# dmkozh/stellar-core

Measured on AMD Instinct MI355X. Metric: ed25519 verifies/sec @1M batch (1/8 GPU) + p50 latency @1k batch, higher is better.
Workload: dtype u32

## Files before the change

stellar-core_amd/csrc/ge25519.h:

```cpp
#pragma once

#include "fe25519.h"



struct ge_p2 { fe X, Y, Z; };
struct ge_p3 { fe X, Y, Z, T; };
struct ge_p1p1 { fe X, Y, Z, T; };
struct ge_cached { fe YpX, YmX, Z, T2d; };
struct ge_precomp { fe ypx, ymx, xy2d; };

SV_HD void ge_p2_identity(ge_p2& p) {
  fe_0(p.X);
  fe_1(p.Y);
  fe_1(p.Z);
}

SV_HD void ge_dbl(ge_p1p1& r, const fe& X, const fe& Y, const fe& Z) {
  fe XX, YY, ZZ2, A, AA;
  fe_add(A, X, Y);
  fe_sq(AA, A);
  fe_sq(XX, X);
  fe_sq(YY, Y);
  fe_sq2(ZZ2, Z);
  fe_add(r.Y, YY, XX);
  fe_sub(r.Z, YY, XX);
  fe_sub4(r.X, AA, r.Y);
  fe_sub4(r.T, ZZ2, r.Z);
  fe_weak_even(r.T);
}

SV_HD void ge_p1p1_convert(ge_p3& r, const ge_p1p1& p, bool wantT) {
  {
    fe19 y19;
    fe_premul19(y19, p.Y);
    if (wantT) fe_mul_g19(r.T, p.X, p.Y, y19);
    fe_mul_g19(r.Y, p.Z, p.Y, y19);
  }
  fe19 t19;
  fe_premul19(t19, p.T);
  fe_mul_g19(r.X, p.X, p.T, t19);
  fe_mul_g19(r.Z, p.Z, p.T, t19);
}

SV_HD void ge_p1p1_to_p2(ge_p2& r, const ge_p1p1& p) {
  ge_p3 t;
  ge_p1p1_convert(t, p, false);
  r.X = t.X;
  r.Y = t.Y;
  r.Z = t.Z;
}

SV_HD void ge_p1p1_to_p3(ge_p3& r, const ge_p1p1& p) { ge_p1p1_convert(r, p, true); }

SV_HD void ge_p1p1_to_p3_opt(ge_p3& r, const ge_p1p1& p, bool wantT) { ge_p1p1_convert(r, p, wantT); }

SV_HD void ge_add_preswapped(ge_p1p1& r, const ge_p3& p, const fe& qa, const fe& qb, const fe& qZ,
                             const fe& qT2d, bool neg, bool zone) {
  fe t0, t1, PP, MM, TT, ZZ2, zp, zm;
  fe_mul(TT, p.T, qT2d);
  if (zone) {
    fe_add(ZZ2, p.Z, p.Z);
    fe_weak(ZZ2);
  } else {
    fe_mul2(ZZ2, p.Z, qZ);
  }
  fe_add(t0, p.Y, p.X);
  fe_sub(t1, p.Y, p.X);
  fe_mul(PP, t0, qa);
  fe_mul(MM, t1, qb);
  fe_sub(r.X, PP, MM);
  fe_add(r.Y, PP, MM);
  fe_add(zp, ZZ2, TT);
  fe_sub(zm, ZZ2, TT);
  SV_UNROLL for (int i = 0; i < 10; ++i) {
    r.Z.v[i] = neg ? zm.v[i] : zp.v[i];
    r.T.v[i] = neg ? zp.v[i] : zm.v[i];
  }
}

SV_HD void ge_p3_to_cached(ge_cached& c, const ge_p3& p) {
  fe d2;
  fe_const_2d(d2);
  fe_add(c.YpX, p.Y, p.X);
  fe_sub(c.YmX, p.Y, p.X);
  c.Z = p.Z;
  fe_mul(c.T2d, p.T, d2);
}

SV_HD void ge_cached_identity(ge_cached& c) {
  fe_1(c.YpX);
  fe_1(c.YmX);
  fe_1(c.Z);
  fe_0(c.T2d);
}

SV_HD bool ge_frombytes_finish(ge_p3& h, const fe& u, const fe& v, const uint32_t w[8], bool negate) {
  fe vxx, chk, chk2, xs, sq;
  fe_sq(vxx, h.X);
  fe_mul(vxx, vxx, v);
  fe_sub(chk, vxx, u);
  fe_add(chk2, vxx, u);
  const bool m_ok = fe_iszero(chk);
  const bool p_ok = fe_iszero(chk2);
  fe_const_sqrtm1(sq);
  fe_mul(xs, h.X, sq);
  fe_cmov(h.X, xs, !m_ok);
  const uint32_t sign = w[7] >> 31;
  fe nx;
  fe_neg(nx, h.X);
  const bool flip = negate ? (fe_isnegative(h.X) == sign) : (fe_isnegative(h.X) != sign);
  fe_cmov(h.X, nx, flip);
  fe_weak(h.X);
  fe_mul(h.T, h.X, h.Y);
  return m_ok || p_ok;
}

SV_COLD bool ge_frombytes(ge_p3& h, const uint32_t w[8], bool negate) {
  fe u, v, v3, one, d;
  fe_1(one);
  fe_const_d(d);
  fe_frombytes(h.Y, w);
  fe_1(h.Z);
  fe_sq(u, h.Y);
  fe_mul(v, u, d);
  fe_sub(u, u, one);
  fe_weak(u);
  fe_add(v, v, one);
  fe_weak(v);
  fe_sq(v3, v);
  fe_mul(v3, v3, v);
  fe_sq(h.X, v3);
  fe_mul(h.X, h.X, v);
  fe_mul(h.X, h.X, u);
  fe_pow22523(h.X, h.X);
  fe_mul(h.X, h.X, v3);
  fe_mul(h.X, h.X, u);
  return ge_frombytes_finish(h, u, v, w, negate);
}

SV_COLD void ge_p2_tobytes_zinv(uint32_t out[8], const fe& X, const fe& Y, const fe& zi) {
  fe x, y;
  fe_mul(x, X, zi);
  fe_mul(y, Y, zi);
  fe_tobytes(out, y);
  out[7] ^= fe_isnegative(x) << 31;
}

SV_COLD void ge_p2_tobytes(uint32_t out[8], const fe& X, const fe& Y, const fe& Z) {
  fe zi;
  fe_invert(zi, Z);
  ge_p2_tobytes_zinv(out, X, Y, zi);
}
```

stellar-core_amd/csrc/sv_kernels.hip:

```cpp
#include <hip/hip_runtime.h>

#include <atomic>

#include "verify_core.h"
#include "quad.h"
#include "sv_kparams.h"
#include "keytab.h"
#include "launch.h"

#define SV_BLOCK 256
#define SV_WAVES_PER_SIMD 2
#ifndef SV_QUAD_WAVES
#define SV_QUAD_WAVES 3
#endif
#ifndef SV_MAIN_WAVES
#define SV_MAIN_WAVES 3
#endif

#define SV_DBG_TRIVIAL_PAIR 1u
#define SV_DBG_MAX_WINDOWS 2u
#define SV_DBG_PREP_ONLY 8u
#define SV_DBG_KEY_COLLIDE 16u
#define SV_DBG_DROP_HANDOVER 0x80u
__device__ __forceinline__ int sv_wave_windows(int wl, uint32_t dbg) {
// ... 85 lines not shown
      ks = (uint32_t)s;
      break;
    }
  }
  t.kslot[li] = ks;
}

__global__ __launch_bounds__(SV_BLOCK, SV_PREP_WAVES) void sv_keybuild_kernel(sv_cparams c) {
  const sv_ktparams& t = c.kt;
  const uint32_t nb = t.count[0];
  const uint64_t i = (uint64_t)blockIdx.x * blockDim.x + threadIdx.x;
  const uint32_t lane = threadIdx.x & 63u;
  if (i - lane >= nb) return;
  const bool active = i < nb;
  const uint32_t s = t.builders[active ? i : nb - 1];
  sv_u4* e = t.store + (uint64_t)s * SV_KT_QUADS;
  uint32_t A[8];
  sv_unpack2(A, e + SV_KT_TQUADS);
  bool ok = sv_point_canonical(A) && !sv_small_order(A);
  ge_p3 negA;
  ok = ge_frombytes(negA, A, true) && ok;
  sv_build_ltab(e, negA);
  if (active) e[SV_KT_TQUADS + 2] = sv_u4{ok ? 1u : 0u, 0u, 0u, 0u};
}

template <int MODE, bool KT, bool DF = false>
__global__ __launch_bounds__(SV_BLOCK, SV_PREP_WAVES) void sv_prep_kernel(sv_cparams c) {
  static_assert(!(KT && DF), "decode-first runs without per-key tables");
  const sv_kparams& p = c.k;
  const uint32_t lane = threadIdx.x & 63u;
  const uint64_t li = (uint64_t)blockIdx.x * blockDim.x + threadIdx.x;
  if (li - lane >= c.cnt) return;
  const bool active = li < c.cnt;
  const uint64_t ii = c.start + (active ? li : c.cnt - 1);
#ifdef SV_DIAG_PREP_ALIAS
  sv_u4* tabA = p.ws + (li & (uint64_t)(SV_DIAG_PREP_ALIAS - 1)) * SV_SLOT_QUADS_L;
#else
  sv_u4* tabA = p.ws + li * SV_SLOT_QUADS_L;
#endif
  sv_u4* tabR = tabA + SV_ATAB_ENTRIES * SV_LTAB_QUADS;
#ifdef SV_PHASE_PROF
  unsigned long long t_prev = __builtin_amdgcn_s_memtime();
#endif
  uint32_t A[8], S[8], hram[16], R[8];
  sv_lat lat;
  bool ok;
  uint32_t ks = SV_KT_NONE;
  if (DF) {
    sv_unpack2(A, p.pk + 2 * ii);
    sv_unpack2(R, p.sig + 4 * ii);
    bool dok;
    {
      ge_p3 negA;
      dok = ge_frombytes(negA, A, true);
      sv_build_ltab(tabA, negA);
    }
    {
      ge_p3 negR;
      dok = ge_frombytes(negR, R, true) && dok;
      sv_build_ltab(tabR, negR);
    }
    sv_load_rest_and_hash<MODE>(p, ii, A, R, S, hram);
    ok = sc_is_canonical(S) && !sv_small_order(R) && sv_point_canonical(R) && sv_point_canonical(A) &&
         !sv_small_order(A) && dok;
    uint32_t h[8];
    sc_reduce512(h, hram);
    sc_lattice_reduce(lat, h, (p.dbg & SV_DBG_TRIVIAL_PAIR) != 0);
  } else {
#ifdef SV_PHASE_PROF
  {
    uint32_t M[8];
    sv_unpack2(A, p.pk + 2 * ii);
    sv_unpack2(R, p.sig + 4 * ii);
    sv_unpack2(S, p.sig + 4 * ii + 2);
    sv_unpack2(M, (const sv_u4*)(p.msg) + 2 * ii);
    asm volatile("s_waitcnt vmcnt(0)" ::: "memory");
    SV_PHASE(5);
    sha512_ram32(hram, R, A, M);
  }
#else
  sv_load_and_hash<MODE>(p, ii, A, S, hram);
  sv_unpack2(R, p.sig + 4 * ii);
#endif
  SV_PHASE(0);
  int a_status = -1;
  if (KT) {
    ks = c.kt.kslot[active ? li : c.cnt - 1];
    bool hit = false;
    uint32_t st = 0;
    if (ks != SV_KT_NONE) {
      const sv_u4* e = c.kt.store + (uint64_t)ks * SV_KT_QUADS + SV_KT_TQUADS;
      const sv_u4 k0 = e[0], k1 = e[1], k2 = e[2];
      hit = k0.x == A[0] && k0.y == A[1] && k0.z == A[2] && k0.w == A[3] && k1.x == A[4] && k1.y == A[5] &&
            k1.z == A[6] && k1.w == A[7];
      st = k2.x;
    }
    if (__ballot(!hit) == 0) a_status = (int)(st & 1u);
    else ks = SV_KT_NONE;
  }
#ifdef SV_PHASE_PROF
  ok = sc_is_canonical(S) && !sv_small_order(R) && sv_point_canonical(A) && !sv_small_order(A) &&
            sv_point_canonical(R);
  ge_p3 negA, negR;
  ok = ge_frombytes(negA, A, true) && ok;
  ok = ge_frombytes(negR, R, true) && ok;
  SV_PHASE(1);
  {
    uint32_t h[8];
    sc_reduce512(h, hram);
    sc_lattice_reduce(lat, h, (p.dbg & SV_DBG_TRIVIAL_PAIR) != 0);
  }
  SV_PHASE(2);
  sv_build_ltab(tabA, negA);
  sv_build_ltab(tabR, negR);
  SV_PHASE(3);
#else
  ok = sv_lat_pre(lat, A, R, S, hram, tabA, tabR, (p.dbg & SV_DBG_TRIVIAL_PAIR) != 0, a_status);
#endif
  }
  const int W = sv_wave_windows(sv_lat_windows(lat.bits), p.dbg);
  sv_lat_digits D;
  sv_lat_prepare(D, lat, S, W);
  const uint32_t flags = (D.rneg ? SV_REC_RNEG : 0u) | (D.top8A ? SV_REC_TOP8A : 0u) |
                         (D.top8R ? SV_REC_TOP8R : 0u) | (ok ? SV_REC_OK : 0u);
  uint32_t rw[4 * SV_REC_QUADS];
  SV_UNROLL for (int k = 0; k < 4 * SV_REC_QUADS; ++k) rw[k] = 0u;
  SV_UNROLL for (int k = 0; k < 8; ++k) {
    rw[k] = D.dA[k];
    rw[8 + k] = D.dR[k];
  }
  SV_UNROLL for (int k = 0; k < SV_LB_DIGITS; ++k) {
    rw[16 + k] = (uint32_t)D.dB0[k];
    rw[16 + SV_LB_DIGITS + k] = (uint32_t)D.dB1[k];
  }
  rw[16 + 2 * SV_LB_DIGITS] = flags;
  rw[16 + 2 * SV_LB_DIGITS + 1] = ks;
  sv_u4* r = c.rec + li * SV_REC_QUADS;
  SV_UNROLL for (int k = 0; k < SV_REC_QUADS; ++k) r[k] = sv_u4{rw[4 * k], rw[4 * k + 1], rw[4 * k + 2], rw[4 * k + 3]};
  if (lane == 0) c.wmax[li >> 6] = (uint32_t)W;
  SV_PHASE(4);
}

__device__ __forceinline__ int32_t sv_nibble(uint32_t word, int p) {
  return (int32_t)__builtin_amdgcn_sbfe((int)word, (unsigned)(4 * (p & 7)), 4u);
}
__device__ sv_u4 sv_ident_lentry[SV_LTAB_QUADS] = {{1u, 0u, 0u, 0u}, {0u, 0u, 0u, 0u}, {0u, 0u, 1u, 0u},
                                                    {0u, 0u, 0u, 0u}, {0u, 0u, 0u, 0u}, {1u, 0u, 0u, 0u},
                                                    {0u, 0u, 0u, 0u}, {0u, 0u, 0u, 0u}, {0u, 0u, 0u, 0u},
                                                    {0u, 0u, 0u, 0u}};
__device__ __forceinline__ const sv_u4* sv_lentry_at(const sv_u4* tab, int32_t d) {
  if (d == 0) return sv_ident_lentry;
  return tab + (d < 0 ? -d : d) * SV_LTAB_QUADS;
}
__device__ __forceinline__ void sv_main_scalarmult(ge_p3& P, const uint32_t* rw, uint32_t flags, int W,
                                                   const sv_u4* tabA, const sv_u4* tabR, const sv_u4* btab0,
                                                   const sv_u4* btab1, sv_u4* stage) {
#if defined(__HIP_DEVICE_COMPILE__)
  const bool top8A = (flags & SV_REC_TOP8A) != 0, top8R = (flags & SV_REC_TOP8R) != 0;
  const bool rneg = (flags & SV_REC_RNEG) != 0;
  uint32_t curA = rw[7], curR = rw[15], nxtA = rw[6], nxtR = rw[14];
  ge_p1p1 Q;
  {
    int32_t dA = top8A ? 8 : sv_nibble(curA, 63), dR = top8R ? 8 : sv_nibble(curR, 63);
    if (rneg) dR = -dR;
    fe qa, qb, qz, qt;
    asm volatile("s_waitcnt lgkmcnt(0)" ::: "memory");
    sv_stage_lentry(stage, sv_lentry_at(tabA, dA));
    asm volatile("s_waitcnt vmcnt(0)" ::: "memory");
    sv_load_lentry(qa, qb, qz, qt, stage + __lane_id(), 64, dA < 0);
    asm volatile("s_waitcnt lgkmcnt(0)" ::: "memory");
    sv_stage_lentry(stage, sv_lentry_at(tabR, dR));
    fe_sub(P.X, qa, qb);
    fe_add(P.Y, qa, qb);
    fe_add(P.Z, qz, qz);
    fe di, nt;
    fe_const_dinv(di);
    fe_mul(P.T, qt, di);
    fe_neg(nt, P.T);
    SV_UNROLL for (int i = 0; i < 10; ++i) P.T.v[i] = dA < 0 ? nt.v[i] : P.T.v[i];
    fe_weak(P.X);
    fe_weak(P.Y);
    fe_weak(P.Z);
    fe_weak(P.T);
    asm volatile("s_waitcnt vmcnt(0)" ::: "memory");
    sv_load_lentry(qa, qb, qz, qt, stage + __lane_id(), 64, dR < 0);
    ge_add_preswapped(Q, P, qa, qb, qz, qt, dR < 0, false);
    ge_p1p1_to_p3_opt(P, Q, false);
  }
  SV_NOUNROLL for (int w = W - 2; w >= 0; --w) {
    const int pos = w + 64 - W;
    if ((pos & 7) == 7 && w != W - 1) {
      curA = nxtA;
      curR = nxtR;
      const int k = (pos >> 3) - 1;
      if (k >= 0) {
        nxtA = rw[k];
        nxtR = rw[8 + k];
      }
    }
    int32_t dA = sv_nibble(curA, pos), dR = sv_nibble(curR, pos);
    if (w == W - 1) {
      if (top8A) dA = 8;
      if (top8R) dR = 8;
    }
    if (rneg) dR = -dR;
    const bool bwin = w % SV_LB_WIN == 0 && w / SV_LB_WIN < SV_LB_DIGITS;
    int32_t dB0 = 0, dB1 = 0;
    if (bwin) {
      dB0 = (int32_t)rw[16 + w / SV_LB_WIN];
      dB1 = (int32_t)rw[16 + SV_LB_DIGITS + w / SV_LB_WIN];
#ifdef SV_DIAG_BTAB_ALIAS
      dB0 %= SV_DIAG_BTAB_ALIAS;
      dB1 %= SV_DIAG_BTAB_ALIAS;
#endif
    }
    const int nsteps = bwin ? 8 : 6;
    const int s0 = (w == W - 1) ? 4 : 0;
    asm volatile("s_waitcnt lgkmcnt(0)" ::: "memory");
    sv_stage_lentry(stage, sv_lentry_at(tabA, dA));
    SV_NOUNROLL for (int s = s0; s < nsteps; ++s) {
      if (s < 4) {
        ge_dbl(Q, P.X, P.Y, P.Z);
      } else {
        fe qa, qb, qz, qt;
        bool neg;
        const bool zone = s >= 6;
        asm volatile("s_waitcnt vmcnt(0)" ::: "memory");
        if (!zone) {
          neg = (s == 4 ? dA : dR) < 0;
          sv_load_lentry(qa, qb, qz, qt, stage + __lane_id(), 64, neg);
          if (s == 4 || bwin) {
            asm volatile("s_waitcnt lgkmcnt(0)" ::: "memory");
            if (s == 4) sv_stage_lentry(stage, sv_lentry_at(tabR, dR));
            else sv_stage_bentry(stage, btab0, dB0);
          }
        } else {
          neg = (s == 6 ? dB0 : dB1) < 0;
          fe_1(qz);
          const sv_u4* st = stage + __lane_id();
          sv_load_fe3(qa, st, 64);
          sv_load_fe3(qb, st + 3 * 64, 64);
          sv_load_fe3(qt, st + 6 * 64, 64);
          if (s == 6) {
            asm volatile("s_waitcnt lgkmcnt(0)" ::: "memory");
            sv_stage_bentry(stage, btab1, dB1);
          }
        }
        ge_add_preswapped(Q, P, qa, qb, qz, qt, neg, zone);
      }
      ge_p1p1_to_p3_opt(P, Q, s + 1 >= 4 && s + 1 < nsteps);
    }
  }
#endif
}

template <bool KT>
__global__ __launch_bounds__(SV_BLOCK, SV_MAIN_WAVES) void sv_main_kernel(sv_cparams c) {
  const sv_kparams& p = c.k;
  __shared__ sv_u4 s_stage[SV_BLOCK / 64][SV_LTAB_QUADS * 64];
  const uint32_t lane = threadIdx.x & 63u;
  sv_u4* stage = s_stage[threadIdx.x >> 6];
  const uint64_t gtid = (uint64_t)blockIdx.x * blockDim.x + threadIdx.x;
  const sv_u4* btab0 = p.btab;
  const sv_u4* btab1 = p.btab + SV_LBTAB_ENTRIES * SV_BTAB_QUADS;
  const uint64_t stride = (uint64_t)gridDim.x * blockDim.x;
  for (uint64_t base = gtid - lane; base < c.cnt; base += stride) {
    const uint64_t li = base + lane;
    const bool active = li < c.cnt;
#ifdef SV_DIAG_TAB_ALIAS
    const sv_u4* slot = p.ws + (li & (uint64_t)(SV_DIAG_TAB_ALIAS - 1)) * SV_SLOT_QUADS_L;
#else
    const sv_u4* slot = p.ws + li * SV_SLOT_QUADS_L;
#endif
    const sv_u4* tabR = slot + SV_ATAB_ENTRIES * SV_LTAB_QUADS;
    const uint32_t* rw = (const uint32_t*)(c.rec + li * SV_REC_QUADS);
    const uint32_t flags = rw[16 + 2 * SV_LB_DIGITS];
    const sv_u4* tabA = slot;
    if (KT) {
      const uint32_t ks = rw[16 + 2 * SV_LB_DIGITS + 1];
      if (ks != SV_KT_NONE) tabA = c.kt.store + (uint64_t)ks * SV_KT_QUADS;
    }
    const bool pre_ok = (flags & SV_REC_OK) != 0;
    const int W = (int)__builtin_amdgcn_readfirstlane(c.wmax[li >> 6]);
    ge_p3 P;
    sv_main_scalarmult(P, rw, flags, W, tabA, tabR, btab0, btab1, stage);
    const bool ok = pre_ok && sv_is_identity(P) && active;
    if (active) p.verdict[c.start + li] = ok ? 1 : 0;
    const uint64_t mask = __ballot(ok);
    if (p.bitmap != nullptr && lane == 0) p.bitmap[(c.start + base) >> 6] = mask;
  }
}

#define SV_QENT_DW 40

__device__ __forceinline__ void qd_load_cached(fe& o, const uint32_t* ent, uint32_t role, bool neg) {
  const uint32_t comp = role == 0 ? 3u : role == 1 ? 2u : ((role == 2) != neg ? 0u : 1u);
  const uint32_t* src = ent + 10 * comp;
  SV_UNROLL for (int k = 0; k < 10; ++k) o.v[k] = src[k];
}
__device__ __forceinline__ void qd_load_affine(fe& o, const sv_u4* ent, uint32_t role, bool neg) {
  const uint32_t comp = role == 0 ? 2u : ((role == 2) != neg ? 0u : 1u);
  const sv_u4* src = ent + 3 * comp;
  const sv_u4 a = src[0], b = src[1], c = src[2];
  o.v[0] = a.x; o.v[1] = a.y; o.v[2] = a.z; o.v[3] = a.w;
  o.v[4] = b.x; o.v[5] = b.y; o.v[6] = b.z; o.v[7] = b.w;
  o.v[8] = c.x; o.v[9] = c.y;
  if (role == 1) fe_1(o);
}

#define SV_OSIGS 8

__device__ __forceinline__ uint32_t oc_from_hi(uint32_t v) {
  return (uint32_t)__builtin_amdgcn_mov_dpp((int)v, 0x104, 0xf, 0xf, false);
}
__device__ __forceinline__ void fe_from_hi(fe& o, const fe& f) {
  SV_UNROLL for (int i = 0; i < 10; ++i) o.v[i] = oc_from_hi(f.v[i]);
}

#define SV_OCTET_BLOCK 128
#define SV_OCTET_BLOCK_HI 192
#ifndef SV_OCT_HI_DIV
#define SV_OCT_HI_DIV 6
#endif
#ifndef SV_OCT_HI_DIV_WIDE
#define SV_OCT_HI_DIV_WIDE 4
#endif
#define SV_OCT_HI_PRE 20
__device__ __forceinline__ int sv_oct_hi_windows(int W, uint32_t dbg) {
  const int div = (dbg & SV_KP_OCT_HI_WIDE) ? SV_OCT_HI_DIV_WIDE : SV_OCT_HI_DIV;
  int h = (W + div / 2) / div;
  h = h < 1 ? 1 : (h > W ? W : h);
  return W - h < SV_OCT_HI_PRE ? 0 : h;
}
enum { SV_OF_PT = 0, SV_OF_TAB, SV_OF_DIG, SV_OF_PB, SV_OF_PHI, SV_OF_N };
__device__ __forceinline__ void sv_oflag_set(uint32_t* f, bool good = true) {
  __builtin_amdgcn_fence(__ATOMIC_RELEASE, "workgroup");
  if ((threadIdx.x & 63u) == 0) __hip_atomic_store(f, good ? 1u : 2u, __ATOMIC_RELAXED, __HIP_MEMORY_SCOPE_WORKGROUP);
}
__device__ __forceinline__ bool sv_oflag_wait(uint32_t* f) {
  uint32_t v = 0;
  for (uint32_t it = 0; it < (1u << 24); ++it) {
    v = __builtin_amdgcn_readfirstlane(__hip_atomic_load(f, __ATOMIC_RELAXED, __HIP_MEMORY_SCOPE_WORKGROUP));
    if (v != 0) break;
    __builtin_amdgcn_s_sleep(1);
  }
  __builtin_amdgcn_fence(__ATOMIC_ACQUIRE, "workgroup");
  return v == 1;
}

#define SV_OCTET_TAB_BYTES (SV_OSIGS * 2 * SV_ATAB_ENTRIES * SV_QENT_DW * 4)
#define SV_OCTET_LDS_BYTES(MSG, HI) (((HI) ? 2 : 1) * SV_OCTET_TAB_BYTES + ((MSG) ? SV_OSIGS * SV_MSG_CAP : 0))
__device__ __forceinline__ void sv_oct_build_table(uint32_t* tab, const ge_p3& Pt, const qd_role& q, uint32_t role) {
  ge_cached c1, ce;
  ge_p3_to_cached(c1, Pt);
  ge_cached_identity(ce);
  const bool store = role == 0;
  if (store) sv_store_lentry((sv_u4*)tab, ce);
  if (store) sv_store_lentry((sv_u4*)(tab + SV_QENT_DW), c1);
  fe mine;
  fe_pick4(mine, q, c1.T2d, c1.Z, c1.YpX, c1.YmX);
  ge_p3 P3 = Pt;
  SV_NOUNROLL for (int e = 2; e < SV_ATAB_ENTRIES; ++e) {
    qd_add(P3, mine, q, false, true);
    ge_p3_to_cached(ce, P3);
    if (store) sv_store_lentry((sv_u4*)(tab + e * SV_QENT_DW), ce);
  }
}
template <int MODE, bool MSG, bool HI>
__global__ __launch_bounds__(HI ? SV_OCTET_BLOCK_HI : SV_OCTET_BLOCK, 1) void sv_octet_kernel(sv_kparams p) {
  extern __shared__ __attribute__((aligned(16))) uint32_t s_dyn[];
  static_assert(SV_OCTET_TAB_BYTES % 16 == 0, "the message windows follow the tables at a 16-byte boundary");
  uint32_t(*s_tab)[2][SV_ATAB_ENTRIES][SV_QENT_DW] = (uint32_t(*)[2][SV_ATAB_ENTRIES][SV_QENT_DW])s_dyn;
  uint32_t(*s_tabh)[2][SV_ATAB_ENTRIES][SV_QENT_DW] =
      (uint32_t(*)[2][SV_ATAB_ENTRIES][SV_QENT_DW])(s_dyn + SV_OCTET_TAB_BYTES / 4);
  __builtin_amdgcn_s_setprio(3);
  const uint32_t lane = threadIdx.x & 63u;
  const uint32_t role = lane & 3u, half = (lane >> 2) & 1u, sl = lane >> 3;
  const qd_role q{role == 1, role == 2, role == 3};
  const uint64_t i = (uint64_t)blockIdx.x * SV_OSIGS + sl;
  const bool active = i < p.n;
  const uint64_t ii = active ? i : p.n - 1;
  __shared__ uint32_t s_dok[SV_OSIGS];
  const uint32_t wv = (uint32_t)__builtin_amdgcn_readfirstlane(threadIdx.x >> 6);
  const bool dec_wave = wv == 1;
  const bool hi_wave = HI && wv == 2;
  __shared__ uint32_t s_pt[HI ? SV_OSIGS : 1][2][40];
  __shared__ uint32_t s_hd[HI ? SV_OSIGS : 1][2][9];
  __shared__ int32_t s_win[2];
  __shared__ uint32_t s_phi[HI ? SV_OSIGS : 1][2][SV_QENT_DW];
  __shared__ uint32_t s_oflag[HI ? SV_OF_N : 1];
  if (HI) {
    if (threadIdx.x < SV_OF_N) s_oflag[threadIdx.x] = 0;
    __syncthreads();
  }
  if (hi_wave) {
    bool good = sv_oflag_wait(&s_oflag[SV_OF_PT]);
    fe h;
    {
      const uint32_t* src = &s_pt[sl][half][10 * role];
      SV_UNROLL for (int k = 0; k < 10; ++k) h.v[k] = src[k];
    }
    SV_NOUNROLL for (int k = 0; k < 4 * SV_OCT_HI_PRE; ++k) qo_dbl(h, q);
    good = sv_oflag_wait(&s_oflag[SV_OF_DIG]) && good;
    const int W = s_win[0], Wlo = s_win[1];
    if (Wlo < W) {
      SV_NOUNROLL for (int k = 4 * SV_OCT_HI_PRE; k < 4 * Wlo; ++k) qo_dbl(h, q);
      ge_p3 Q;
      qo_expand(Q, h);
      uint32_t* tabh = &s_tabh[sl][half][0][0];
      sv_oct_build_table(tabh, Q, q, role);
      __builtin_amdgcn_fence(__ATOMIC_RELEASE, "wavefront");
      __builtin_amdgcn_wave_barrier();
      __builtin_amdgcn_fence(__ATOMIC_ACQUIRE, "wavefront");
      uint32_t dg[8];
// ... 676 lines not shown
```

stellar-core_amd/csrc/verify_core.h:

```cpp
#pragma once

#include "ge25519.h"
#include "lattice.h"
#include "sc25519.h"
#include "sha512_dev.h"

struct __attribute__((aligned(16))) sv_u4 {
  uint32_t x, y, z, w;
};

#define SV_B_BITS 16
#define SV_BTAB_ENTRIES ((1 << (SV_B_BITS - 1)) + 1)
#define SV_BTAB_STRIDE 36
#define SV_BTAB_DWORDS (SV_BTAB_ENTRIES * SV_BTAB_STRIDE)
#define SV_ATAB_ENTRIES 9
#define SV_ATAB_QUADS 11
#define SV_SLOT_QUADS_W (SV_ATAB_ENTRIES * SV_ATAB_QUADS)
#define SV_LTAB_QUADS 10
#define SV_SLOT_QUADS_L (2 * SV_ATAB_ENTRIES * SV_LTAB_QUADS)
#define SV_SLOT_QUADS (SV_SLOT_QUADS_W > SV_SLOT_QUADS_L ? SV_SLOT_QUADS_W : SV_SLOT_QUADS_L)

SV_HD bool sv_small_order(const uint32_t s[8]) {
  const uint32_t bl[7][8] = {
      {0x00000000u, 0x00000000u, 0x00000000u, 0x00000000u, 0x00000000u, 0x00000000u, 0x00000000u, 0x00000000u},
      {0x00000001u, 0x00000000u, 0x00000000u, 0x00000000u, 0x00000000u, 0x00000000u, 0x00000000u, 0x00000000u},
      {0x8f95e826u, 0xb027b2c2u, 0x89f4c345u, 0xf098eff2u, 0x05acdfd5u, 0x3933c6d3u, 0x880238b1u, 0x05fc536du},
      {0x706a17c7u, 0x4fd84d3du, 0x760b3cbau, 0x0f67100du, 0xfa53202au, 0xc6cc392cu, 0x77fdc74eu, 0x7a03ac92u},
      {0xffffffecu, 0xffffffffu, 0xffffffffu, 0xffffffffu, 0xffffffffu, 0xffffffffu, 0xffffffffu, 0x7fffffffu},
      {0xffffffedu, 0xffffffffu, 0xffffffffu, 0xffffffffu, 0xffffffffu, 0xffffffffu, 0xffffffffu, 0x7fffffffu},
      {0xffffffeeu, 0xffffffffu, 0xffffffffu, 0xffffffffu, 0xffffffffu, 0xffffffffu, 0xffffffffu, 0x7fffffffu}};
  bool hit = false;
  SV_UNROLL for (int k = 0; k < 7; ++k) {
    uint32_t diff = (s[7] & 0x7fffffffu) ^ bl[k][7];
    SV_UNROLL for (int i = 0; i < 7; ++i) diff |= s[i] ^ bl[k][i];
    hit |= (diff == 0);
  }
  return hit;
}

SV_HD bool sv_point_canonical(const uint32_t s[8]) {
  uint32_t ones = (s[7] & 0x7fffffffu) ^ 0x7fffffffu;
  SV_UNROLL for (int i = 1; i < 7; ++i) ones |= s[i] ^ 0xffffffffu;
  return !(ones == 0 && s[0] >= 0xffffffedu);
}

SV_HD void sv_store_fe3(sv_u4* p, int qstride, const fe& f) {
  p[0] = sv_u4{f.v[0], f.v[1], f.v[2], f.v[3]};
  p[qstride] = sv_u4{f.v[4], f.v[5], f.v[6], f.v[7]};
  p[2 * qstride] = sv_u4{f.v[8], f.v[9], 0u, 0u};
}
SV_HD void sv_load_fe3(fe& f, const sv_u4* p, int qstride) {
  const sv_u4 a = p[0], b = p[qstride], c = p[2 * qstride];
  f.v[0] = a.x; f.v[1] = a.y; f.v[2] = a.z; f.v[3] = a.w;
  f.v[4] = b.x; f.v[5] = b.y; f.v[6] = b.z; f.v[7] = b.w;
  f.v[8] = c.x; f.v[9] = c.y;
}

SV_HD void sv_store_fe_pair(sv_u4* p, int qstride, const fe& a, const fe& b) {
  p[0] = sv_u4{a.v[0], a.v[1], a.v[2], a.v[3]};
  p[qstride] = sv_u4{a.v[4], a.v[5], a.v[6], a.v[7]};
  p[2 * qstride] = sv_u4{a.v[8], a.v[9], b.v[0], b.v[1]};
  p[3 * qstride] = sv_u4{b.v[2], b.v[3], b.v[4], b.v[5]};
  p[4 * qstride] = sv_u4{b.v[6], b.v[7], b.v[8], b.v[9]};
}
SV_HD void sv_load_fe_pair(fe& a, fe& b, const sv_u4* p, int qstride) {
  const sv_u4 q0 = p[0], q1 = p[qstride], q2 = p[2 * qstride], q3 = p[3 * qstride], q4 = p[4 * qstride];
  a.v[0] = q0.x; a.v[1] = q0.y; a.v[2] = q0.z; a.v[3] = q0.w;
  a.v[4] = q1.x; a.v[5] = q1.y; a.v[6] = q1.z; a.v[7] = q1.w;
  a.v[8] = q2.x; a.v[9] = q2.y; b.v[0] = q2.z; b.v[1] = q2.w;
  b.v[2] = q3.x; b.v[3] = q3.y; b.v[4] = q3.z; b.v[5] = q3.w;
  b.v[6] = q4.x; b.v[7] = q4.y; b.v[8] = q4.z; b.v[9] = q4.w;
}

SV_HD void sv_store_cached(sv_u4* slot, int qstride, int e, const ge_cached& c) {
  sv_u4* base = slot + e * SV_ATAB_QUADS * qstride;
  sv_store_fe3(base, qstride, c.YpX);
  sv_store_fe3(base + 3 * qstride, qstride, c.YmX);
  sv_store_fe_pair(base + 6 * qstride, qstride, c.Z, c.T2d);
}

SV_COLD void sv_build_atab(sv_u4* slot, int qstride, const ge_p3& negA) {
  ge_cached c1, ce;
  ge_p3_to_cached(c1, negA);
  ge_cached_identity(ce);
  sv_store_cached(slot, qstride, 0, ce);
  sv_store_cached(slot, qstride, 1, c1);
  ge_p3 P3 = negA;
  ge_p1p1 Q;
  SV_NOUNROLL for (int e = 2; e < SV_ATAB_ENTRIES; ++e) {
    ge_add_preswapped(Q, P3, c1.YpX, c1.YmX, c1.Z, c1.T2d, false, false);
    ge_p1p1_to_p3(P3, Q);
    ge_p3_to_cached(ce, P3);
    sv_store_cached(slot, qstride, e, ce);
  }
}

#define SV_BTAB_QUADS (SV_BTAB_STRIDE / 4)

#if defined(__HIP_DEVICE_COMPILE__)
#define SV_GLDS(SRC, OFF, STAGE, ROW)                                                                 \
  __builtin_amdgcn_global_load_lds(                                                                   \
      (const void*)(SRC),                                                                             \
      (__attribute__((address_space(3))) void*)((char*)((STAGE) + (ROW) * 64) - 16 * (OFF)), 16, 16 * (OFF), 0)
SV_HD void sv_stage_bentry(sv_u4* stageB, const sv_u4* btab, int32_t d) {
  const bool neg = d < 0;
  const sv_u4* e = btab + (neg ? -d : d) * SV_BTAB_QUADS;
  const sv_u4* ea = e + (neg ? 3 : 0);
  const sv_u4* eb = e + (neg ? 0 : 3);
  SV_GLDS(ea, 0, stageB, 0); SV_GLDS(ea, 1, stageB, 1); SV_GLDS(ea, 2, stageB, 2);
  SV_GLDS(eb, 0, stageB, 3); SV_GLDS(eb, 1, stageB, 4); SV_GLDS(eb, 2, stageB, 5);
  SV_GLDS(e, 6, stageB, 6); SV_GLDS(e, 7, stageB, 7); SV_GLDS(e, 8, stageB, 8);
  static_assert(SV_BTAB_QUADS == 9, "entry size");
}
#endif

SV_HD void sv_double_scalarmult(ge_p3& P, const ge_p3& negA, const uint32_t h[8], const uint32_t S[8],
                                sv_u4* slot, int qstride, const sv_u4* btab) {
  sv_build_atab(slot, qstride, negA);
  uint32_t da[8], db[8];
  sc_digits_r16(da, h);
  sc_digits_r65536(db, S);

  fe_0(P.X); fe_1(P.Y); fe_1(P.Z); fe_0(P.T);
  ge_p1p1 Q;
  SV_NOUNROLL for (int w = 63; w >= 0; --w) {
    const int nsteps = (w & (SV_B_BITS / 4 - 1)) ? 5 : 6;
    const int32_t dA = sc_pop_top(da, 4);
    const int32_t dB = nsteps == 6 ? sc_pop_top(db, SV_B_BITS) : 0;
    SV_NOUNROLL for (int s = 0; s < nsteps; ++s) {
      if (s < 4) {
        ge_dbl(Q, P.X, P.Y, P.Z);
      } else {
        fe qa, qb, qz, qt;
        bool neg;
        const bool zone = s == 5;
        if (!zone) {
          neg = dA < 0;
          const sv_u4* e = slot + (neg ? -dA : dA) * SV_ATAB_QUADS * qstride;
          sv_load_fe3(qa, e + (neg ? 3 : 0) * qstride, qstride);
          sv_load_fe3(qb, e + (neg ? 0 : 3) * qstride, qstride);
          sv_load_fe_pair(qz, qt, e + 6 * qstride, qstride);
        } else {
          neg = dB < 0;
          fe_1(qz);
          const sv_u4* e = btab + (neg ? -dB : dB) * SV_BTAB_QUADS;
          sv_load_fe3(qa, e + (neg ? 3 : 0), 1);
          sv_load_fe3(qb, e + (neg ? 0 : 3), 1);
          sv_load_fe3(qt, e + 6, 1);
        }
        ge_add_preswapped(Q, P, qa, qb, qz, qt, neg, zone);
      }
      ge_p1p1_to_p3_opt(P, Q, s + 1 >= 4 && s + 1 < nsteps);
    }
  }
}

SV_HD void sv_double_scalarmult_encode(uint32_t enc[8], const ge_p3& negA, const uint32_t h[8],
                                       const uint32_t S[8], sv_u4* slot, int qstride,
                                       const sv_u4* btab) {
  ge_p3 P;
  sv_double_scalarmult(P, negA, h, S, slot, qstride, btab);
  ge_p2_tobytes(enc, P.X, P.Y, P.Z);
}

SV_HD bool sv_verify_pre(ge_p3& P, const uint32_t A[8], const sv_u4* Rp, const uint32_t S[8],
                         const uint32_t hram[16], sv_u4* slot, int qstride, const sv_u4* btab) {
  bool ok;
  {
    uint32_t R[8];
    const sv_u4 r0 = Rp[0], r1 = Rp[1];
    R[0] = r0.x; R[1] = r0.y; R[2] = r0.z; R[3] = r0.w;
    R[4] = r1.x; R[5] = r1.y; R[6] = r1.z; R[7] = r1.w;
    ok = sc_is_canonical(S) && !sv_small_order(R) && sv_point_canonical(A) && !sv_small_order(A);
  }
  ge_p3 negA;
  ok = ge_frombytes(negA, A, true) && ok;
  uint32_t h[8];
  sc_reduce512(h, hram);
  uint32_t Sc[8];
  SV_UNROLL for (int i = 0; i < 8; ++i) Sc[i] = S[i];
  Sc[7] &= 0x1fffffffu;
  sv_double_scalarmult(P, negA, h, Sc, slot, qstride, btab);
  if (!ok) fe_1(P.Z);
  return ok;
}

SV_HD bool sv_encode_matches(const fe& X, const fe& Y, const fe& zi, const sv_u4* Rp) {
  uint32_t enc[8];
  ge_p2_tobytes_zinv(enc, X, Y, zi);
  const sv_u4 r0 = Rp[0], r1 = Rp[1];
  const uint32_t diff = (enc[0] ^ r0.x) | (enc[1] ^ r0.y) | (enc[2] ^ r0.z) | (enc[3] ^ r0.w) |
                        (enc[4] ^ r1.x) | (enc[5] ^ r1.y) | (enc[6] ^ r1.z) | (enc[7] ^ r1.w);
  return diff == 0;
}

SV_HD bool sv_verify_core(const uint32_t A[8], const sv_u4* Rp, const uint32_t S[8],
                          const uint32_t hram[16], sv_u4* slot, int qstride, const sv_u4* btab) {
  ge_p3 P;
  const bool ok = sv_verify_pre(P, A, Rp, S, hram, slot, qstride, btab);
  fe zi;
  fe_invert(zi, P.Z);
  return sv_encode_matches(P.X, P.Y, zi, Rp) && ok;
}

SV_HD void sv_btab_entry(uint32_t out[SV_BTAB_STRIDE], int e) {
  const uint32_t benc[8] = {0x66666658u, 0x66666666u, 0x66666666u, 0x66666666u,
                            0x66666666u, 0x66666666u, 0x66666666u, 0x66666666u};
  ge_p3 B, acc;
  ge_frombytes(B, benc, false);
  ge_cached bc;
  ge_p3_to_cached(bc, B);
  fe_0(acc.X); fe_1(acc.Y); fe_1(acc.Z); fe_0(acc.T);
  ge_p1p1 Q;
  for (int bit = SV_B_BITS - 1; bit >= 0; --bit) {
    ge_dbl(Q, acc.X, acc.Y, acc.Z);
    ge_p1p1_to_p3(acc, Q);
    if ((e >> bit) & 1) {
      ge_add_preswapped(Q, acc, bc.YpX, bc.YmX, bc.Z, bc.T2d, false, false);
      ge_p1p1_to_p3(acc, Q);
    }
  }
  fe zi, x, y, xy, d2, ypx, ymx, xy2d;
  fe_invert(zi, acc.Z);
  fe_mul(x, acc.X, zi);
  fe_mul(y, acc.Y, zi);
  fe_mul(xy, x, y);
  fe_const_2d(d2);
  fe_mul(xy2d, xy, d2);
  fe_add(ypx, y, x);
  fe_weak(ypx);
  fe_sub(ymx, y, x);
  fe_weak(ymx);
  for (int i = 0; i < SV_BTAB_STRIDE; ++i) out[i] = 0;
  for (int i = 0; i < 10; ++i) {
    out[i] = ypx.v[i];
    out[12 + i] = ymx.v[i];
    out[24 + i] = xy2d.v[i];
  }
}


template <int NW>
SV_HD void sha512_words(uint32_t out[16], const uint32_t* in) {
  uint64_t st[8], w[16];
  sha512_init(st);
  SV_UNROLL for (int t = 0; t < 16; ++t) w[t] = 0;
  SV_UNROLL for (int t = 0; t < NW / 2; ++t) w[t] = sv_be64(in[2 * t], in[2 * t + 1]);
  w[NW / 2] = 0x8000000000000000ULL;
  w[15] = (uint64_t)NW * 32;
  sha512_compress(st, w);
  sha512_digest_le(out, st);
}

SV_HD void sc_muladd(uint32_t s[8], const uint32_t a[8], const uint32_t b[8], const uint32_t c[8]) {
  uint32_t x[16];
  SV_UNROLL for (int i = 0; i < 16; ++i) x[i] = 0;
  SV_UNROLL for (int i = 0; i < 8; ++i) {
    uint64_t carry = 0;
    SV_UNROLL for (int j = 0; j < 8; ++j) {
      const uint64_t t = (uint64_t)a[i] * b[j] + x[i + j] + carry;
      x[i + j] = (uint32_t)t;
      carry = t >> 32;
    }
    x[i + 8] = (uint32_t)carry;
// ... 32 lines not shown
  uint32_t S[8];
  sc_muladd(S, h, a, r);
  SV_UNROLL for (int i = 0; i < 8; ++i) { sig[i] = enc[i]; sig[8 + i] = S[i]; }
}

#ifndef SV_LB_BITS
#define SV_LB_BITS 16
#endif
static_assert(SV_LB_BITS % 4 == 0 && 128 % SV_LB_BITS == 0 && SV_LB_BITS <= 16, "base-point digit radix");
#define SV_LB_WIN (SV_LB_BITS / 4)
#define SV_LB_DIGITS (128 / SV_LB_BITS)
#define SV_LBTAB_ENTRIES ((1 << (SV_LB_BITS - 1)) + 1)

SV_HD void sv_btab_entry_shift(uint32_t out[SV_BTAB_STRIDE], int e, int shift) {
  const uint32_t benc[8] = {0x66666658u, 0x66666666u, 0x66666666u, 0x66666666u,
                            0x66666666u, 0x66666666u, 0x66666666u, 0x66666666u};
  ge_p3 B, acc;
  ge_frombytes(B, benc, false);
  ge_p1p1 Q;
  for (int i = 0; i < shift; ++i) {
    ge_dbl(Q, B.X, B.Y, B.Z);
    ge_p1p1_to_p3(B, Q);
  }
  ge_cached bc;
  ge_p3_to_cached(bc, B);
  fe_0(acc.X); fe_1(acc.Y); fe_1(acc.Z); fe_0(acc.T);
  for (int bit = SV_LB_BITS - 1; bit >= 0; --bit) {
    ge_dbl(Q, acc.X, acc.Y, acc.Z);
    ge_p1p1_to_p3(acc, Q);
    if ((e >> bit) & 1) {
      ge_add_preswapped(Q, acc, bc.YpX, bc.YmX, bc.Z, bc.T2d, false, false);
      ge_p1p1_to_p3(acc, Q);
    }
  }
  fe zi, x, y, xy, d2, ypx, ymx, xy2d;
  fe_invert(zi, acc.Z);
  fe_mul(x, acc.X, zi);
  fe_mul(y, acc.Y, zi);
  fe_mul(xy, x, y);
  fe_const_2d(d2);
  fe_mul(xy2d, xy, d2);
  fe_add(ypx, y, x);
  fe_weak(ypx);
  fe_sub(ymx, y, x);
  fe_weak(ymx);
  for (int i = 0; i < SV_BTAB_STRIDE; ++i) out[i] = 0;
  for (int i = 0; i < 10; ++i) {
    out[i] = ypx.v[i];
    out[12 + i] = ymx.v[i];
    out[24 + i] = xy2d.v[i];
  }
}

SV_HD void sv_store_lentry(sv_u4* p, const ge_cached& c) {
  uint32_t w[40];
  SV_UNROLL for (int i = 0; i < 10; ++i) {
    w[i] = c.YpX.v[i];
    w[10 + i] = c.YmX.v[i];
    w[20 + i] = c.Z.v[i];
    w[30 + i] = c.T2d.v[i];
  }
  SV_UNROLL for (int q = 0; q < 10; ++q) p[q] = sv_u4{w[4 * q], w[4 * q + 1], w[4 * q + 2], w[4 * q + 3]};
}
SV_HD void sv_load_lentry(fe& qa, fe& qb, fe& qz, fe& qt, const sv_u4* p, int qstride, bool neg) {
  uint32_t w[40];
  SV_UNROLL for (int q = 0; q < 10; ++q) {
    const sv_u4 v = p[q * qstride];
    w[4 * q] = v.x; w[4 * q + 1] = v.y; w[4 * q + 2] = v.z; w[4 * q + 3] = v.w;
  }
  SV_UNROLL for (int i = 0; i < 10; ++i) {
    qa.v[i] = neg ? w[10 + i] : w[i];
    qb.v[i] = neg ? w[i] : w[10 + i];
    qz.v[i] = w[20 + i];
    qt.v[i] = w[30 + i];
  }
}

SV_COLD void sv_build_ltab(sv_u4* tab, const ge_p3& P) {
  ge_cached c1, ce;
  ge_p3_to_cached(c1, P);
  ge_cached_identity(ce);
#if !defined(__HIP_DEVICE_COMPILE__)
  sv_store_lentry(tab, ce);
#endif
  sv_store_lentry(tab + SV_LTAB_QUADS, c1);
  ge_p3 P3 = P;
  ge_p1p1 Q;
  SV_NOUNROLL for (int e = 2; e < SV_ATAB_ENTRIES; ++e) {
    ge_add_preswapped(Q, P3, c1.YpX, c1.YmX, c1.Z, c1.T2d, false, true);
    ge_p1p1_to_p3(P3, Q);
    ge_p3_to_cached(ce, P3);
    sv_store_lentry(tab + e * SV_LTAB_QUADS, ce);
  }
}

SV_HD void sv_digits_shift(uint32_t d[8], int k) {
  SV_NOUNROLL while (k >= 8) {
    SV_UNROLL for (int i = 7; i > 0; --i) d[i] = d[i - 1];
    d[0] = 0;
    k -= 8;
  }
  SV_NOUNROLL for (; k > 0; --k) (void)sc_pop_top(d, 4);
}

struct sv_lat_digits {
  uint32_t dA[8], dR[8];
  int32_t dB0[SV_LB_DIGITS], dB1[SV_LB_DIGITS];
  bool rneg, top8A, top8R;
};

SV_HD void sc_digits_lb(int32_t d0[SV_LB_DIGITS], int32_t d1[SV_LB_DIGITS], const uint32_t x[8]) {
  uint32_t carry = 0;
  SV_UNROLL for (int j = 0; j < 2 * SV_LB_DIGITS; ++j) {
    const int o = j * SV_LB_BITS, q = o >> 5, r = o & 31;
    uint32_t v = ((x[q] >> r) & ((1u << SV_LB_BITS) - 1u)) + carry;
    carry = (v + (1u << (SV_LB_BITS - 1))) >> SV_LB_BITS;
    const int32_t d = (int32_t)v - (int32_t)(carry << SV_LB_BITS);
    if (j < SV_LB_DIGITS) d0[j] = d;
    else d1[j - SV_LB_DIGITS] = d;
  }
}

SV_HD bool sv_lat_bdigits(sv_lat_digits& D, int w, int32_t& dB0, int32_t& dB1) {
  dB0 = dB1 = 0;
  if (w % SV_LB_WIN != 0 || w / SV_LB_WIN >= SV_LB_DIGITS) return false;
  dB0 = D.dB0[SV_LB_DIGITS - 1];
  dB1 = D.dB1[SV_LB_DIGITS - 1];
  SV_UNROLL for (int k = SV_LB_DIGITS - 1; k > 0; --k) {
    D.dB0[k] = D.dB0[k - 1];
    D.dB1[k] = D.dB1[k - 1];
  }
  D.dB0[0] = D.dB1[0] = 0;
  return true;
}

SV_COLD void sv_lat_prepare(sv_lat_digits& D, const sv_lat& lat, const uint32_t S[8], int W) {
  sc_digits_r16(D.dA, lat.c0);
  sc_digits_r16(D.dR, lat.c1);
  if (W < 64) {
    sv_digits_shift(D.dA, 63 - W);
    sv_digits_shift(D.dR, 63 - W);
    D.top8A = sc_pop_top(D.dA, 4) != 0;
    D.top8R = sc_pop_top(D.dR, 4) != 0;
  } else {
    D.top8A = D.top8R = false;
  }
  D.rneg = lat.c1neg;
  uint32_t s[8];
  sc_mul_signed(s, lat.c1, lat.c1neg, S);
  sc_digits_lb(D.dB0, D.dB1, s);
}

#if defined(__HIP_DEVICE_COMPILE__)
SV_HD void sv_stage_lentry(sv_u4* stage, const sv_u4* entry) {
  SV_GLDS(entry, 0, stage, 0); SV_GLDS(entry, 1, stage, 1); SV_GLDS(entry, 2, stage, 2);
  SV_GLDS(entry, 3, stage, 3); SV_GLDS(entry, 4, stage, 4); SV_GLDS(entry, 5, stage, 5);
  SV_GLDS(entry, 6, stage, 6); SV_GLDS(entry, 7, stage, 7); SV_GLDS(entry, 8, stage, 8);
  SV_GLDS(entry, 9, stage, 9);
  static_assert(SV_LTAB_QUADS == 10, "entry size");
}
#endif

SV_HD void sv_lat_scalarmult(ge_p3& P, sv_lat_digits& D, int W, const sv_u4* tabA, const sv_u4* tabR,
                             const sv_u4* btab0, const sv_u4* btab1) {
  fe_0(P.X); fe_1(P.Y); fe_1(P.Z); fe_0(P.T);
  ge_p1p1 Q;
  SV_NOUNROLL for (int w = W - 1; w >= 0; --w) {
    int32_t dA = sc_pop_top(D.dA, 4);
    int32_t dR = sc_pop_top(D.dR, 4);
    if (w == W - 1) {
      if (D.top8A) dA = 8;
      if (D.top8R) dR = 8;
    }
    if (D.rneg) dR = -dR;
    int32_t dB0, dB1;
    const bool bwin = sv_lat_bdigits(D, w, dB0, dB1);
    const int nsteps = bwin ? 8 : 6;
    const int s0 = (w == W - 1) ? 4 : 0;
    SV_NOUNROLL for (int s = s0; s < nsteps; ++s) {
      if (s < 4) {
        ge_dbl(Q, P.X, P.Y, P.Z);
      } else {
        fe qa, qb, qz, qt;
        bool neg;
        const bool zone = s >= 6;
        if (!zone) {
          const int32_t d = s == 4 ? dA : dR;
          neg = d < 0;
          const sv_u4* e = (s == 4 ? tabA : tabR) + (neg ? -d : d) * SV_LTAB_QUADS;
          sv_load_lentry(qa, qb, qz, qt, e, 1, neg);
        } else {
          const int32_t d = s == 6 ? dB0 : dB1;
          neg = d < 0;
          fe_1(qz);
          const sv_u4* e = (s == 6 ? btab0 : btab1) + (neg ? -d : d) * SV_BTAB_QUADS;
          sv_load_fe3(qa, e + (neg ? 3 : 0), 1);
          sv_load_fe3(qb, e + (neg ? 0 : 3), 1);
          sv_load_fe3(qt, e + 6, 1);
        }
        ge_add_preswapped(Q, P, qa, qb, qz, qt, neg, zone);
      }
      ge_p1p1_to_p3_opt(P, Q, s + 1 >= 4 && s + 1 < nsteps);
    }
  }
}

SV_HD bool sv_is_identity(const ge_p3& P) {
  fe d;
  fe_sub(d, P.Y, P.Z);
  return fe_iszero(P.X) && fe_iszero(d);
}

SV_COLD bool sv_lat_pre(sv_lat& lat, const uint32_t A[8], const uint32_t R[8], const uint32_t S[8],
                        const uint32_t hram[16], sv_u4* tabA, sv_u4* tabR, bool trivial = false,
                        int a_status = -1) {
  bool ok = sc_is_canonical(S) && !sv_small_order(R) && sv_point_canonical(R) &&
            (a_status >= 0 ? a_status != 0 : (sv_point_canonical(A) && !sv_small_order(A)));
  uint32_t h[8];
  sc_reduce512(h, hram);
  if (a_status < 0) {
    ge_p3 negA;
    ok = ge_frombytes(negA, A, true) && ok;
    sv_build_ltab(tabA, negA);
  }
  {
    ge_p3 negR;
    ok = ge_frombytes(negR, R, true) && ok;
    sv_build_ltab(tabR, negR);
  }
  sc_lattice_reduce(lat, h, trivial);
  return ok;
}
```

Measured before the change: 108.0 million.

## Pace next-entry LDS DMA staging inside point add and select sign by address

Restructures the table-entry staging in the main scalar-mult loop. Global-to-LDS DMA of the next entry can now be split into groups interleaved between the field multiplies of the point addition, through a callback hook in ge_add_preswapped. With the default of one group it is issued in a single burst as before. The stage base is made wave-uniform via readfirstlane. Sign swaps of ypx/ymx are now done by choosing LDS read addresses instead of swapping the DMA source, which unifies the B-entry staging. The aim is to hide load latency and cut per-entry address and select overhead, at the cost of extra template and fence complexity.

```diff
diff --git a/stellar-core_amd/csrc/ge25519.h b/stellar-core_amd/csrc/ge25519.h
--- a/stellar-core_amd/csrc/ge25519.h
+++ b/stellar-core_amd/csrc/ge25519.h
@@ -55,19 +55,23 @@
 
 SV_HD void ge_p1p1_to_p3_opt(ge_p3& r, const ge_p1p1& p, bool wantT) { ge_p1p1_convert(r, p, wantT); }
 
-SV_HD void ge_add_preswapped(ge_p1p1& r, const ge_p3& p, const fe& qa, const fe& qb, const fe& qZ,
-                             const fe& qT2d, bool neg, bool zone) {
+template <class Between>
+SV_HD void ge_add_preswapped_with(ge_p1p1& r, const ge_p3& p, const fe& qa, const fe& qb, const fe& qZ,
+                                  const fe& qT2d, bool neg, bool zone, Between&& between) {
   fe t0, t1, PP, MM, TT, ZZ2, zp, zm;
   fe_mul(TT, p.T, qT2d);
+  between(1);
   if (zone) {
     fe_add(ZZ2, p.Z, p.Z);
     fe_weak(ZZ2);
   } else {
     fe_mul2(ZZ2, p.Z, qZ);
   }
+  between(2);
   fe_add(t0, p.Y, p.X);
   fe_sub(t1, p.Y, p.X);
   fe_mul(PP, t0, qa);
+  between(3);
   fe_mul(MM, t1, qb);
   fe_sub(r.X, PP, MM);
   fe_add(r.Y, PP, MM);
@@ -77,6 +81,10 @@
     r.Z.v[i] = neg ? zm.v[i] : zp.v[i];
     r.T.v[i] = neg ? zp.v[i] : zm.v[i];
   }
+}
+SV_HD void ge_add_preswapped(ge_p1p1& r, const ge_p3& p, const fe& qa, const fe& qb, const fe& qZ,
+                             const fe& qT2d, bool neg, bool zone) {
+  ge_add_preswapped_with(r, p, qa, qb, qZ, qT2d, neg, zone, [](int) {});
 }
 
 SV_HD void ge_p3_to_cached(ge_cached& c, const ge_p3& p) {
diff --git a/stellar-core_amd/csrc/sv_kernels.hip b/stellar-core_amd/csrc/sv_kernels.hip
--- a/stellar-core_amd/csrc/sv_kernels.hip
+++ b/stellar-core_amd/csrc/sv_kernels.hip
@@ -261,12 +261,51 @@
   if (d == 0) return sv_ident_lentry;
   return tab + (d < 0 ? -d : d) * SV_LTAB_QUADS;
 }
+#ifndef SV_MAIN_DMA_GROUPS
+#define SV_MAIN_DMA_GROUPS 1
+#endif
+#ifndef SV_MAIN_SIGN_BY_ADDR
+#define SV_MAIN_SIGN_BY_ADDR 1
+#endif
+static_assert(SV_MAIN_DMA_GROUPS >= 1 && SV_MAIN_DMA_GROUPS <= 4, "one group per product statement at most");
+#if defined(__HIP_DEVICE_COMPILE__)
+struct sv_next_entry {
+  int nq;
+  const sv_u4* e;
+};
+template <int G, int g>
+__device__ __forceinline__ void sv_stage_group(uint32_t sbase, const sv_next_entry& n) {
+  static_assert(SV_BTAB_QUADS == 9 && SV_LTAB_QUADS == 10, "entry sizes");
+  if (n.nq == 0) return;
+  sv_stage_quads<9 * g / G, 9 * (g + 1) / G>(sbase, n.e);
+  if (g == G - 1 && n.nq == SV_LTAB_QUADS) sv_stage_quads<9, 10>(sbase, n.e);
+}
+template <int G>
+__device__ __forceinline__ void sv_stage_paced(uint32_t sbase, const sv_next_entry& n, int k) {
+  if (G > 1 && k > 0) SV_FENCE();
+  if (k == 0) sv_stage_group<G, 0>(sbase, n);
+  if (G > 1 && k == 4 * 1 / G) sv_stage_group<G, 1 % G>(sbase, n);
+  if (G > 2 && k == 4 * 2 / G) sv_stage_group<G, 2 % G>(sbase, n);
+  if (G > 3 && k == 4 * 3 / G) sv_stage_group<G, 3 % G>(sbase, n);
+  if (G > 1 && k > 0) SV_FENCE();
+}
+__device__ __forceinline__ void sv_main_load_lentry(fe& qa, fe& qb, fe& qz, fe& qt, const sv_u4* st, bool neg) {
+#if SV_MAIN_SIGN_BY_ADDR
+  sv_load_lentry_stage(qa, qb, qz, qt, st, neg);
+#else
+  sv_load_lentry(qa, qb, qz, qt, st, 64, neg);
+#endif
+}
+#endif
 __device__ __forceinline__ void sv_main_scalarmult(ge_p3& P, const uint32_t* rw, uint32_t flags, int W,
                                                    const sv_u4* tabA, const sv_u4* tabR, const sv_u4* btab0,
-                                                   const sv_u4* btab1, sv_u4* stage) {
+                                                   const sv_u4* btab1, const sv_u4* stage) {
 #if defined(__HIP_DEVICE_COMPILE__)
+  constexpr int G = SV_MAIN_DMA_GROUPS;
+  const uint32_t sbase = sv_stage_sbase(stage);
   const bool top8A = (flags & SV_REC_TOP8A) != 0, top8R = (flags & SV_REC_TOP8R) != 0;
   const bool rneg = (flags & SV_REC_RNEG) != 0;
+  const sv_u4* st = stage + __lane_id();
   uint32_t curA = rw[7], curR = rw[15], nxtA = rw[6], nxtR = rw[14];
   ge_p1p1 Q;
   {
@@ -274,17 +313,21 @@
     if (rneg) dR = -dR;
     fe qa, qb, qz, qt;
     asm volatile("s_waitcnt lgkmcnt(0)" ::: "memory");
-    sv_stage_lentry(stage, sv_lentry_at(tabA, dA));
+    sv_stage_lentry(sbase, sv_lentry_at(tabA, dA));
     asm volatile("s_waitcnt vmcnt(0)" ::: "memory");
-    sv_load_lentry(qa, qb, qz, qt, stage + __lane_id(), 64, dA < 0);
+    sv_main_load_lentry(qa, qb, qz, qt, st, dA < 0);
     asm volatile("s_waitcnt lgkmcnt(0)" ::: "memory");
-    sv_stage_lentry(stage, sv_lentry_at(tabR, dR));
+    const sv_next_entry nR{SV_LTAB_QUADS, sv_lentry_at(tabR, dR)};
+    sv_stage_paced<G>(sbase, nR, 0);
     fe_sub(P.X, qa, qb);
     fe_add(P.Y, qa, qb);
     fe_add(P.Z, qz, qz);
     fe di, nt;
     fe_const_dinv(di);
+    sv_stage_paced<G>(sbase, nR, 1);
+    sv_stage_paced<G>(sbase, nR, 2);
     fe_mul(P.T, qt, di);
+    sv_stage_paced<G>(sbase, nR, 3);
     fe_neg(nt, P.T);
     SV_UNROLL for (int i = 0; i < 10; ++i) P.T.v[i] = dA < 0 ? nt.v[i] : P.T.v[i];
     fe_weak(P.X);
@@ -292,7 +335,7 @@
     fe_weak(P.Z);
     fe_weak(P.T);
     asm volatile("s_waitcnt vmcnt(0)" ::: "memory");
-    sv_load_lentry(qa, qb, qz, qt, stage + __lane_id(), 64, dR < 0);
+    sv_main_load_lentry(qa, qb, qz, qt, st, dR < 0);
     ge_add_preswapped(Q, P, qa, qb, qz, qt, dR < 0, false);
     ge_p1p1_to_p3_opt(P, Q, false);
   }
@@ -326,7 +369,7 @@
     const int nsteps = bwin ? 8 : 6;
     const int s0 = (w == W - 1) ? 4 : 0;
     asm volatile("s_waitcnt lgkmcnt(0)" ::: "memory");
-    sv_stage_lentry(stage, sv_lentry_at(tabA, dA));
+    sv_stage_lentry(sbase, sv_lentry_at(tabA, dA));
     SV_NOUNROLL for (int s = s0; s < nsteps; ++s) {
       if (s < 4) {
         ge_dbl(Q, P.X, P.Y, P.Z);
@@ -334,28 +377,35 @@
         fe qa, qb, qz, qt;
         bool neg;
         const bool zone = s >= 6;
+        sv_next_entry nx;
+        nx.nq = 0;
         asm volatile("s_waitcnt vmcnt(0)" ::: "memory");
         if (!zone) {
           neg = (s == 4 ? dA : dR) < 0;
-          sv_load_lentry(qa, qb, qz, qt, stage + __lane_id(), 64, neg);
-          if (s == 4 || bwin) {
-            asm volatile("s_waitcnt lgkmcnt(0)" ::: "memory");
-            if (s == 4) sv_stage_lentry(stage, sv_lentry_at(tabR, dR));
-            else sv_stage_bentry(stage, btab0, dB0);
+          sv_main_load_lentry(qa, qb, qz, qt, st, neg);
+          if (s == 4) {
+            nx.nq = SV_LTAB_QUADS;
+            nx.e = sv_lentry_at(tabR, dR);
+          } else if (bwin) {
+            nx.nq = SV_BTAB_QUADS;
+            nx.e = sv_bentry_at(btab0, dB0);
           }
         } else {
           neg = (s == 6 ? dB0 : dB1) < 0;
           fe_1(qz);
-          const sv_u4* st = stage + __lane_id();
-          sv_load_fe3(qa, st, 64);
-          sv_load_fe3(qb, st + 3 * 64, 64);
-          sv_load_fe3(qt, st + 6 * 64, 64);
+          sv_load_bentry_stage(qa, qb, qt, st, neg);
           if (s == 6) {
-            asm volatile("s_waitcnt lgkmcnt(0)" ::: "memory");
-            sv_stage_bentry(stage, btab1, dB1);
+            nx.nq = SV_BTAB_QUADS;
+            nx.e = sv_bentry_at(btab1, dB1);
           }
         }
-        ge_add_preswapped(Q, P, qa, qb, qz, qt, neg, zone);
+        if (nx.nq != 0) {
+          asm volatile("s_waitcnt lgkmcnt(0)" ::: "memory");
+          sv_stage_paced<G>(sbase, nx, 0);
+        }
+        ge_add_preswapped_with(Q, P, qa, qb, qz, qt, neg, zone, [&](int k) {
+          if (G > 1) sv_stage_paced<G>(sbase, nx, k);
+        });
       }
       ge_p1p1_to_p3_opt(P, Q, s + 1 >= 4 && s + 1 < nsteps);
     }
@@ -368,7 +418,7 @@
   const sv_kparams& p = c.k;
   __shared__ sv_u4 s_stage[SV_BLOCK / 64][SV_LTAB_QUADS * 64];
   const uint32_t lane = threadIdx.x & 63u;
-  sv_u4* stage = s_stage[threadIdx.x >> 6];
+  const sv_u4* stage = s_stage[threadIdx.x >> 6];
   const uint64_t gtid = (uint64_t)blockIdx.x * blockDim.x + threadIdx.x;
   const sv_u4* btab0 = p.btab;
   const sv_u4* btab1 = p.btab + SV_LBTAB_ENTRIES * SV_BTAB_QUADS;
diff --git a/stellar-core_amd/csrc/verify_core.h b/stellar-core_amd/csrc/verify_core.h
--- a/stellar-core_amd/csrc/verify_core.h
+++ b/stellar-core_amd/csrc/verify_core.h
@@ -98,18 +98,26 @@
 #define SV_BTAB_QUADS (SV_BTAB_STRIDE / 4)
 
 #if defined(__HIP_DEVICE_COMPILE__)
-#define SV_GLDS(SRC, OFF, STAGE, ROW)                                                                 \
+#define SV_GLDS(SRC, OFF, SBASE, ROW)                                                                 \
   __builtin_amdgcn_global_load_lds(                                                                   \
       (const void*)(SRC),                                                                             \
-      (__attribute__((address_space(3))) void*)((char*)((STAGE) + (ROW) * 64) - 16 * (OFF)), 16, 16 * (OFF), 0)
-SV_HD void sv_stage_bentry(sv_u4* stageB, const sv_u4* btab, int32_t d) {
-  const bool neg = d < 0;
-  const sv_u4* e = btab + (neg ? -d : d) * SV_BTAB_QUADS;
-  const sv_u4* ea = e + (neg ? 3 : 0);
-  const sv_u4* eb = e + (neg ? 0 : 3);
-  SV_GLDS(ea, 0, stageB, 0); SV_GLDS(ea, 1, stageB, 1); SV_GLDS(ea, 2, stageB, 2);
-  SV_GLDS(eb, 0, stageB, 3); SV_GLDS(eb, 1, stageB, 4); SV_GLDS(eb, 2, stageB, 5);
-  SV_GLDS(e, 6, stageB, 6); SV_GLDS(e, 7, stageB, 7); SV_GLDS(e, 8, stageB, 8);
+      (__attribute__((address_space(3))) void*)(uint32_t)((SBASE) + 1024u * (ROW) - 16u * (OFF)), 16, 16 * (OFF), 0)
+SV_HD uint32_t sv_stage_sbase(const sv_u4* stage) {
+  return __builtin_amdgcn_readfirstlane((uint32_t)(uintptr_t)(__attribute__((address_space(3))) const void*)stage);
+}
+template <int Q0, int Q1>
+SV_HD void sv_stage_quads(uint32_t sbase, const sv_u4* entry) {
+#define SV_SQ(Q) if (Q0 <= (Q) && (Q) < Q1) SV_GLDS(entry, Q, sbase, Q)
+  SV_SQ(0); SV_SQ(1); SV_SQ(2); SV_SQ(3); SV_SQ(4); SV_SQ(5); SV_SQ(6); SV_SQ(7); SV_SQ(8); SV_SQ(9);
+#undef SV_SQ
+  static_assert(Q1 <= 10, "rows of the stage");
+}
+SV_HD const sv_u4* sv_bentry_at(const sv_u4* btab, int32_t d) { return btab + (d < 0 ? -d : d) * SV_BTAB_QUADS; }
+SV_HD void sv_load_bentry_stage(fe& qa, fe& qb, fe& qt, const sv_u4* st, bool neg) {
+  const int o = neg ? 3 * 64 : 0;
+  sv_load_fe3(qa, st + o, 64);
+  sv_load_fe3(qb, st + (3 * 64 - o), 64);
+  sv_load_fe3(qt, st + 6 * 64, 64);
   static_assert(SV_BTAB_QUADS == 9, "entry size");
 }
 #endif
@@ -448,12 +456,27 @@
 }
 
 #if defined(__HIP_DEVICE_COMPILE__)
-SV_HD void sv_stage_lentry(sv_u4* stage, const sv_u4* entry) {
-  SV_GLDS(entry, 0, stage, 0); SV_GLDS(entry, 1, stage, 1); SV_GLDS(entry, 2, stage, 2);
-  SV_GLDS(entry, 3, stage, 3); SV_GLDS(entry, 4, stage, 4); SV_GLDS(entry, 5, stage, 5);
-  SV_GLDS(entry, 6, stage, 6); SV_GLDS(entry, 7, stage, 7); SV_GLDS(entry, 8, stage, 8);
-  SV_GLDS(entry, 9, stage, 9);
+SV_HD void sv_stage_lentry(uint32_t sbase, const sv_u4* entry) {
+  sv_stage_quads<0, SV_LTAB_QUADS>(sbase, entry);
   static_assert(SV_LTAB_QUADS == 10, "entry size");
+}
+SV_HD void sv_load_lentry_stage(fe& qa, fe& qb, fe& qz, fe& qt, const sv_u4* st, bool neg) {
+  struct __attribute__((aligned(8))) u2 {
+    uint32_t x, y;
+  };
+  const char* b = (const char*)st;
+  const uint32_t o0 = neg ? 2056u : 0u, o1 = neg ? 3064u : 0u;
+  const u2* a0 = (const u2*)(b + o0);
+  const u2* a1 = (const u2*)(b + 8 + o1);
+  const u2* b0 = (const u2*)(b + 2056 - o0);
+  const u2* b1 = (const u2*)(b + 3072 - o1);
+  SV_UNROLL for (int i = 0; i < 5; ++i) {
+    const u2 va = (i & 1) ? a1[128 * (i >> 1)] : a0[128 * (i >> 1)];
+    const u2 vb = (i & 1) ? b1[128 * (i >> 1)] : b0[128 * (i >> 1)];
+    qa.v[2 * i] = va.x; qa.v[2 * i + 1] = va.y;
+    qb.v[2 * i] = vb.x; qb.v[2 * i + 1] = vb.y;
+  }
+  sv_load_fe_pair(qz, qt, st + 5 * 64, 64);
 }
 #endif
 
```

Result: faster. 109.8 million (median of 6 runs) (+1.6%).
